# mahfuzalhasan/WaveFormer

Measured on AMD Instinct MI355X. Metric: 128³×4 volumes/sec fwd (1/2/4/8 MI355X) + Dice Δ vs reference, higher is better.
Workload: dtype bf16x3; 1 GPU; MultiscaleTransformer (WaveFormer encoder) forward, 128^3x4 crops; global_batch=8, per_gpu_batch=8, precision=bf16x3, parallelism=replicas x1 (no data-path collective), hip_graph=True

## Files before the change

waveformer_amd/csrc/pw2.hip:

```cpp
#include <algorithm>

#include "gemm_common.hpp"

namespace wf {

namespace pw2 {
constexpr int K = 96, N = 384, KS = K / 32, NT = N / 16;
constexpr int RB = K * 2;
constexpr int PLANE = N * RB;
}

__device__ __forceinline__ int pw2_chunk(int n, int o) {
  const int f = (0x1E >> (2 * ((n >> 2) & 3))) & 3;
  return (o & ~3) | ((o & 3) ^ f);
}

template <int P, int NW>
__global__ __launch_bounds__(64 * NW, 1) void pw2_res_kernel(GemmArgs g) {
  using namespace pw2;
  constexpr bool SPLIT = P == PREC_SPLIT;
  constexpr int NPL = SPLIT ? 2 : 1;
  extern __shared__ __attribute__((aligned(16))) unsigned char smem[];
  float* ew = reinterpret_cast<float*>(smem + NPL * PLANE);
  float* eb = ew + N;
  float* bs = eb + N;
  float* aw = bs + N;
  float* ab = aw + K;
  const int tid = threadIdx.x, lane = tid & 63, wid = tid >> 6;
  const int l15 = lane & 15, g4 = lane >> 4;

  for (int it = tid; it < NPL * N * (K / 8); it += 64 * NW) {
    const int pr = it / (K / 8), o = it - pr * (K / 8);
    const int n = pr % N;
    *reinterpret_cast<bf16x8*>(smem + pr * RB + 16 * pw2_chunk(n, o)) =
        *reinterpret_cast<const bf16x8*>(g.w + (int64_t)pr * K + 8 * o);
  }
  for (int i = tid; i < N; i += 64 * NW) {
    ew[i] = 0.5f * g.e_ln_w[i];
    eb[i] = 0.5f * g.e_ln_b[i];
    bs[i] = g.bias ? g.bias[i] : 0.f;
  }
  const bool aln = g.a_ln == LN_GIVEN;
  for (int i = tid; i < K; i += 64 * NW) {
    aw[i] = aln ? g.a_ln_w[i] : 1.f;
    ab[i] = aln ? g.a_ln_b[i] : 0.f;
  }
  __syncthreads();

  const int M = (int)g.M;
  const int ntiles = (M + 15) >> 4;
  const float* xa = reinterpret_cast<const float*>(g.a_src);
  f32x4 an[KS][2];
  float mn = 0.f, rn = 1.f;
  auto aload = [&](int tile) {
    const int row = min(tile * 16 + l15, M - 1);
    const float* p = xa + (int64_t)row * K + 8 * g4;
#pragma unroll
    for (int ks = 0; ks < KS; ++ks) {
      an[ks][0] = *reinterpret_cast<const f32x4*>(p + 32 * ks);
      an[ks][1] = *reinterpret_cast<const f32x4*>(p + 32 * ks + 4);
    }
    if (aln) {
      mn = g.a_stats[2 * row];
      rn = g.a_stats[2 * row + 1];
    }
  };
  int tile = blockIdx.x * NW + wid;
  const int stride = gridDim.x * NW;
  if (tile < ntiles) aload(tile);
  const int wlane = l15 * RB + 16 * ((g4 ^ ((0x1E >> (2 * ((l15 >> 2) & 3))) & 3)));
  for (; tile < ntiles; tile += stride) {
    bf16x8 ah[KS], al[KS];
    const float mu = mn, rs = rn;
#pragma unroll
    for (int ks = 0; ks < KS; ++ks) {
      const int k = 32 * ks + 8 * g4;
#pragma unroll
      for (int hq = 0; hq < 2; ++hq) {
        f32x4 v = an[ks][hq];
        if (aln) {
          const f32x4 lw = *reinterpret_cast<const f32x4*>(aw + k + 4 * hq);
          const f32x4 lb = *reinterpret_cast<const f32x4*>(ab + k + 4 * hq);
          v = (v - mu) * rs * lw + lb;
        }
        uint32_t h0, h1, l0, l1;
        split_pair<P>(v[0], v[1], h0, l0);
        split_pair<P>(v[2], v[3], h1, l1);
        ah[ks][4 * hq] = (short)(h0 & 0xFFFF);
        ah[ks][4 * hq + 1] = (short)(h0 >> 16);
        ah[ks][4 * hq + 2] = (short)(h1 & 0xFFFF);
        ah[ks][4 * hq + 3] = (short)(h1 >> 16);
        al[ks][4 * hq] = (short)(l0 & 0xFFFF);
        al[ks][4 * hq + 1] = (short)(l0 >> 16);
        al[ks][4 * hq + 2] = (short)(l1 & 0xFFFF);
        al[ks][4 * hq + 3] = (short)(l1 >> 16);
      }
    }
    if (tile + stride < ntiles) aload(tile + stride);

    int wb = wlane;
    asm volatile("" : "+v"(wb));
    const unsigned char* Wb = smem + wb;
    f32x4 acc[NT];
#pragma unroll
    for (int t = 0; t < NT; ++t) acc[t] = f32x4{0.f, 0.f, 0.f, 0.f};
#pragma unroll
    for (int ks = 0; ks < KS; ++ks) {
#pragma unroll
      for (int t = 0; t < NT; ++t) {
        const int wo = t * 16 * RB + 64 * ks;
        const bf16x8 bh = *reinterpret_cast<const bf16x8*>(Wb + wo);
        const bf16x8 bl = SPLIT ? *reinterpret_cast<const bf16x8*>(Wb + PLANE + wo) : bh;
        acc[t] = mma3<P>(acc[t], bh, bl, ah[ks], al[ks]);
        if (t % 4 == 3) __builtin_amdgcn_sched_barrier(0);
      }
    }

#pragma unroll
    for (int t = 0; t < NT; ++t) acc[t] += *reinterpret_cast<const f32x4*>(bs + 16 * t + 4 * g4);
    float part[8];
#pragma unroll
    for (int w = 0; w < 8; ++w) part[w] = tile_sum<3>(acc + 3 * w);
    const float mean =
        (((part[0] + part[1]) + (part[2] + part[3])) + ((part[4] + part[5]) + (part[6] + part[7]))) *
        (1.f / N);
#pragma unroll
    for (int w = 0; w < 8; ++w) part[w] = tile_sqdev<3>(acc + 3 * w, mean);
    const float rstd = rsqrtf(
        (((part[0] + part[1]) + (part[2] + part[3])) + ((part[4] + part[5]) + (part[6] + part[7]))) *
            (1.f / N) + g.e_eps);
    const int row = tile * 16 + l15;
    float* o = reinterpret_cast<float*>(g.out) + (int64_t)min(row, M - 1) * g.ldo + 4 * g4;
#pragma unroll
    for (int t = 0; t < NT; ++t) {
      const f32x4 lw = *reinterpret_cast<const f32x4*>(ew + 16 * t + 4 * g4);
      const f32x4 lb = *reinterpret_cast<const f32x4*>(eb + 16 * t + 4 * g4);
      const f32x4 v = gelu_half4((acc[t] - mean) * rstd * lw + lb);
      if (row < M) *reinterpret_cast<f32x4*>(o + 16 * t) = v;
      if (t % 4 == 3) __builtin_amdgcn_sched_barrier(0);
    }
  }
}

int try_launch_pw2_resident(const GemmArgs& g, hipStream_t s) {
  using namespace pw2;
  static const bool off = getenv("WF_PW2_RES") != nullptr && getenv("WF_PW2_RES")[0] == '0';
  if (off || g.epi != EPI_LN_GELU || g.a_map != MAP_IDENTITY || g.a_bf16 || g.a_gelu ||
      !(g.a_ln == LN_NONE || g.a_ln == LN_GIVEN) || g.K != K || g.N != N || g.a_C != K ||
      g.out_bf16 || g.ldo < N || g.ldo % 4 != 0 || (g.prec != PREC_SPLIT && g.prec != PREC_FP16) ||
      g.M < 1 || g.M >= ((int64_t)1 << 31) - 16)
    return 0;
  constexpr int NW = 8;
  const bool split = g.prec == PREC_SPLIT;
  const size_t lds = (size_t)(split ? 2 : 1) * PLANE + (size_t)(3 * N + 2 * K) * 4;
  void (*kern)(GemmArgs) = split ? pw2_res_kernel<PREC_SPLIT, NW> : pw2_res_kernel<PREC_FP16, NW>;
  set_max_lds(reinterpret_cast<const void*>(kern), (int)lds);
  const int64_t ntiles = (g.M + 15) / 16;
  const unsigned gx = (unsigned)std::min<int64_t>(cdiv(ntiles, NW), 256);
  hipLaunchKernelGGL(kern, dim3(gx), dim3(64 * NW), lds, s, g);
  return 1;
}

}
```

waveformer_amd/csrc/gemm.hip:

```cpp
#include "gemm_common.hpp"

namespace wf {

__device__ __forceinline__ void load8(const void* src, int is_bf16, int64_t off, float (&v)[8]) {
  if (is_bf16) load8f<true>(src, off, v);
  else load8f<false>(src, off, v);
}

struct RowSource {
  const GemmArgs& g;
  int64_t pos;
  __device__ RowSource(const GemmArgs& g_, int64_t m) : g(g_), pos(0) {
    if (g.a_map == MAP_WINDOW) {
      const int ws = g.mws;
      const int N = ws * ws * ws;
      const int nWd = g.mD / ws, nWh = g.mH / ws, nWw = g.mW / ws;
      const int64_t bw = m / N;
      const int t = (int)(m - bw * N);
      const int nW = nWd * nWh * nWw;
      const int b = (int)(bw / nW);
      int wi = (int)(bw - (int64_t)b * nW);
      const int wx = wi % nWw;
      wi /= nWw;
      const int wy = wi % nWh;
      const int wz = wi / nWh;
      const int tx = t % ws, ty = (t / ws) % ws, tz = t / (ws * ws);
      pos = (((int64_t)b * g.mD + wz * ws + tz) * g.mH + wy * ws + ty) * g.mW + wx * ws + tx;
    } else if (g.a_map == MAP_MERGE) {
      const int d = g.mD >> 1, h = g.mH >> 1, w = g.mW >> 1;
      int64_t r = m;
      const int x = (int)(r % w);
      r /= w;
      const int y = (int)(r % h);
      r /= h;
      const int z = (int)(r % d);
      const int b = (int)(r / d);
      pos = (((int64_t)b * g.mD + 2 * z) * g.mH + 2 * y) * g.mW + 2 * x;
    } else {
      pos = m;
    }
  }
  __device__ int64_t offset(int k) const {
    if (g.a_map == MAP_MERGE) {
      const int seg = k / g.a_C;
      const int c = k - seg * g.a_C;
      const int o = (g.merge_code >> (4 * seg)) & 0xF;
      const int64_t p = pos + (((int64_t)((o >> 2) & 1) * g.mH + ((o >> 1) & 1)) * g.mW) +
                        (o & 1);
      return p * g.a_C + c;
    }
    return pos * (int64_t)(g.a_C * g.a_nseg) + k;
  }
};

template <int TPR>
__device__ __forceinline__ float tpr_sum(float v) {
#pragma unroll
  for (int o = TPR / 2; o > 0; o >>= 1) v += __shfl_xor(v, o, 64);
  return v;
}

template <int BM, int P>
__global__ __launch_bounds__(256) void gemm_ares_kernel(GemmArgs g) {
  constexpr bool SPLIT = P == PREC_SPLIT;
  extern __shared__ __attribute__((aligned(16))) char smem[];
  constexpr int TPR = 256 / BM;
  constexpr int MT = BM / 16;
  const int K = g.K, N = g.N;
  const int K32 = (K + 31) & ~31;
  const int KP = K32 + 8;
  const int NP = N + 4;
  const size_t abytes = ((size_t)BM * KP * 2 + 15) & ~(size_t)15;
  uint16_t* A = reinterpret_cast<uint16_t*>(smem);
  uint16_t* Alo = reinterpret_cast<uint16_t*>(smem + abytes);
  float* R = reinterpret_cast<float*>(smem + (SPLIT ? 2 : 1) * abytes);
  float* st = R + (size_t)BM * NP;

  const int tid = threadIdx.x, lane = tid & 63, wid = tid >> 6;
  const int64_t m0 = (int64_t)blockIdx.x * BM;

  {
    const int r = tid / TPR, q = tid % TPR;
    const int64_t m = m0 + r;
    const bool mv = m < g.M;
    float mean = 0.f, rstd = 1.f;
    if (g.a_ln == LN_GIVEN) {
      if (mv) {
        mean = g.a_stats[2 * m];
        rstd = g.a_stats[2 * m + 1];
      }
    } else if (g.a_ln == LN_COMPUTE) {
      RowSource rs(g, mv ? m : 0);
      float s = 0.f;
      for (int ch = q; ch < K / 8; ch += TPR) {
        float v[8];
        load8(g.a_src, g.a_bf16, rs.offset(ch * 8), v);
#pragma unroll
        for (int j = 0; j < 8; ++j) s += v[j];
      }
      mean = tpr_sum<TPR>(s) / (float)K;
      float sq = 0.f;
      for (int ch = q; ch < K / 8; ch += TPR) {
        float v[8];
        load8(g.a_src, g.a_bf16, rs.offset(ch * 8), v);
#pragma unroll
        for (int j = 0; j < 8; ++j) {
          const float dlt = v[j] - mean;
          sq += dlt * dlt;
        }
      }
      rstd = rsqrtf(tpr_sum<TPR>(sq) / (float)K + g.a_eps);
    } else if (g.a_ln == LN_PARTIAL) {
      const int np = g.a_np;
      const float* ps = g.a_stats + (mv ? m : 0) * np * 2;
      float s = 0.f;
      for (int c = q; c < np; c += TPR) s += ps[2 * c];
      mean = tpr_sum<TPR>(s) / (float)np;
      const float ng = (float)(K / np);
      float sq = 0.f;
      for (int c = q; c < np; c += TPR) {
        const float d = ps[2 * c] - mean;
        sq += ps[2 * c + 1] + ng * d * d;
      }
      rstd = rsqrtf(tpr_sum<TPR>(sq) / (float)K + g.a_eps);
    }
    if (q == 0) {
      st[2 * r] = mean;
      st[2 * r + 1] = rstd;
    }
  }
  __syncthreads();
  {
    const int KC = K32 / 8;
    for (int item = tid; item < BM * KC; item += 256) {
      const int r = item / KC, ch = item - r * KC;
      const int64_t m = m0 + r;
      bf16x8 o = {0, 0, 0, 0, 0, 0, 0, 0}, olo = {0, 0, 0, 0, 0, 0, 0, 0};
      if (m < g.M && ch * 8 < K) {
        RowSource rs(g, m);
        float v[8];
        load8(g.a_src, g.a_bf16, rs.offset(ch * 8), v);
        if (g.a_ln != LN_NONE) {
          const float mean = st[2 * r], rstd = st[2 * r + 1];
          const f32x4* gw = reinterpret_cast<const f32x4*>(g.a_ln_w + ch * 8);
          const f32x4* gb = reinterpret_cast<const f32x4*>(g.a_ln_b + ch * 8);
          const f32x4 w0 = gw[0], w1 = gw[1], b0 = gb[0], b1 = gb[1];
          const float wv[8] = {w0.x, w0.y, w0.z, w0.w, w1.x, w1.y, w1.z, w1.w};
          const float bv[8] = {b0.x, b0.y, b0.z, b0.w, b1.x, b1.y, b1.z, b1.w};
#pragma unroll
          for (int j = 0; j < 8; ++j) v[j] = (v[j] - mean) * rstd * wv[j] + bv[j];
        }
        if (g.a_gelu) {
          gelu_erf8(v);
        }
#pragma unroll
        for (int j = 0; j < 8; ++j) {
          const uint16_t hi = op_cvt<P>(v[j]);
          o[j] = (short)hi;
          if (SPLIT) olo[j] = op_lo<P>(v[j], hi);
        }
      }
      *reinterpret_cast<bf16x8*>(A + (size_t)r * KP + ch * 8) = o;
      if (SPLIT) *reinterpret_cast<bf16x8*>(Alo + (size_t)r * KP + ch * 8) = olo;
    }
  }
  __syncthreads();

  const int kq = 8 * (lane >> 4);
  for (int n0 = 0; n0 < N; n0 += 64) {
    const int n = n0 + wid * 16 + (lane & 15);
    const bool nv = n < N;
    const uint16_t* wrow = g.w + (int64_t)(nv ? n : 0) * K;
    const uint16_t* wlo = wrow + (int64_t)N * K;
    f32x4 acc[MT];
#pragma unroll
    for (int mt = 0; mt < MT; ++mt) acc[mt] = f32x4{0, 0, 0, 0};
    const bf16x8 z8 = {0, 0, 0, 0, 0, 0, 0, 0};
    bf16x8 bnext = z8, blnext = z8;
    if (nv && kq < K) {
      bnext = *reinterpret_cast<const bf16x8*>(wrow + kq);
      if (SPLIT) blnext = *reinterpret_cast<const bf16x8*>(wlo + kq);
    }
    for (int k0 = 0; k0 < K32; k0 += 32) {
      const bf16x8 b = bnext, bl = blnext;
      bnext = z8;
      blnext = z8;
      if (nv && k0 + 32 + kq < K) {
        bnext = *reinterpret_cast<const bf16x8*>(wrow + k0 + 32 + kq);
        if (SPLIT) blnext = *reinterpret_cast<const bf16x8*>(wlo + k0 + 32 + kq);
      }
#pragma unroll
      for (int mt = 0; mt < MT; ++mt) {
        const size_t aoff = (size_t)(mt * 16 + (lane & 15)) * KP + k0 + kq;
        const bf16x8 a = *reinterpret_cast<const bf16x8*>(A + aoff);
        if (SPLIT) {
          const bf16x8 al = *reinterpret_cast<const bf16x8*>(Alo + aoff);
          acc[mt] = mma32<P>(al, b, acc[mt]);
          acc[mt] = mma32<P>(a, bl, acc[mt]);
        }
        acc[mt] = mma32<P>(a, b, acc[mt]);
      }
    }
    if (nv) {
#pragma unroll
      for (int mt = 0; mt < MT; ++mt)
#pragma unroll
        for (int i = 0; i < 4; ++i) R[(size_t)(mt * 16 + 4 * (lane >> 4) + i) * NP + n] = acc[mt][i];
    }
  }
  __syncthreads();

  const int N4 = N >> 2;
  if (g.epi == EPI_LN_GELU) {
    const int r = tid / TPR, q = tid % TPR;
    float s = 0.f;
    for (int c4 = q; c4 < N4; c4 += TPR) {
      f32x4 v = *reinterpret_cast<const f32x4*>(R + (size_t)r * NP + 4 * c4);
      if (g.bias) v += reinterpret_cast<const f32x4*>(g.bias)[c4];
      s += (v.x + v.y) + (v.z + v.w);
    }
    const float mean = tpr_sum<TPR>(s) / (float)N;
    float sq = 0.f;
    for (int c4 = q; c4 < N4; c4 += TPR) {
      f32x4 v = *reinterpret_cast<const f32x4*>(R + (size_t)r * NP + 4 * c4);
      if (g.bias) v += reinterpret_cast<const f32x4*>(g.bias)[c4];
      v -= mean;
      sq += (v.x * v.x + v.y * v.y) + (v.z * v.z + v.w * v.w);
    }
    const float rstd = rsqrtf(tpr_sum<TPR>(sq) / (float)N + g.e_eps);
    __syncthreads();
    if (q == 0) {
      st[2 * r] = mean;
      st[2 * r + 1] = rstd;
    }
    __syncthreads();
  }
  for (int item = tid; item < BM * N4; item += 256) {
    const int r = item / N4, c4 = item - r * N4;
    const int64_t m = m0 + r;
    if (m >= g.M) continue;
    f32x4 v = *reinterpret_cast<const f32x4*>(R + (size_t)r * NP + 4 * c4);
    if (g.bias) v += reinterpret_cast<const f32x4*>(g.bias)[c4];
    if (g.epi == EPI_LN_GELU) {
      const f32x4 lw = reinterpret_cast<const f32x4*>(g.e_ln_w)[c4];
      const f32x4 lb = reinterpret_cast<const f32x4*>(g.e_ln_b)[c4];
      v = (v - st[2 * r]) * st[2 * r + 1] * lw + lb;
      v = gelu_erf4(v);
    } else if (g.epi == EPI_RESID) {
      const f32x4 xr = reinterpret_cast<const f32x4*>(g.r_x + m * (int64_t)N)[c4];
      const float bs = g.r_scale ? g.r_scale[m / g.rows_per_sample] : 1.f;
      float mean = 0.f, rstd = 1.f;
      if (g.r_stats) {
        mean = g.r_stats[2 * m];
        rstd = g.r_stats[2 * m + 1];
      }
      v = resid_epilogue(v, xr, mean, rstd, g.r_ln_w + 4 * c4, g.r_ln_b + 4 * c4, bs,
                         g.r_stats != nullptr);
    }
    store4(g.out, g.out_bf16 != 0, m * g.ldo, 4 * c4, v);
  }
}

static size_t gemm_lds_bytes(int BM, int K, int N, bool split) {
  const size_t K32 = (size_t)((K + 31) & ~31);
  const size_t a = ((size_t)BM * (K32 + 8) * 2 + 15) & ~(size_t)15;
  return (split ? 2 : 1) * a + (size_t)BM * (N + 4) * 4 + (size_t)BM * 2 * 4;
}

int launch_gemm(const GemmArgs& g, hipStream_t s, const char* who) {
  if (g.K <= 0 || g.K % 8 != 0) return fail(WF_E_SHAPE, std::string(who) + ": K must be a positive multiple of 8");
  if (g.N <= 0 || g.N % 4 != 0) return fail(WF_E_SHAPE, std::string(who) + ": N must be a positive multiple of 4");
  if (g.a_C % 8 != 0) return fail(WF_E_SHAPE, std::string(who) + ": channels must be a multiple of 8");
  if (g.M <= 0) return WF_OK;
  if (g.o_pstats) {
    if (g.epi == EPI_STORE && !g.out_bf16 && !g.a_bf16 && try_launch_gemm_kc(g, s))
      return check_launch(who);
    return fail(WF_E_SHAPE, std::string(who) + ": LN-partial epilogue needs the gemm_kc shape");
  }
  if (try_launch_gemm_lnw(g, s)) return check_launch(who);
  if (try_launch_gemm_rows(g, s, true)) return check_launch(who);
  if (try_launch_gemm_kc(g, s)) return check_launch(who);
  const bool split = g.prec == PREC_SPLIT;
  int BM = 64;
  while (BM > 16 && gemm_lds_bytes(BM, g.K, g.N, split) > 80 * 1024) BM >>= 1;
  const size_t lds = gemm_lds_bytes(BM, g.K, g.N, split);
  if (lds > 160 * 1024) return fail(WF_E_SHAPE, std::string(who) + ": K/N too large for the LDS tile");
  const unsigned blocks = (unsigned)cdiv(g.M, BM);
  auto go = [&](auto kern) {
    if (lds > 64 * 1024)
      set_max_lds(reinterpret_cast<const void*>(kern), (int)lds);
    hipLaunchKernelGGL(kern, dim3(blocks), dim3(256), lds, s, g);
  };
  gemm_with_prec(g.prec, false, [&](auto P, auto) {
    switch (BM) {
      case 64: go(gemm_ares_kernel<64, P()>); break;
      case 32: go(gemm_ares_kernel<32, P()>); break;
      default: go(gemm_ares_kernel<16, P()>); break;
    }
  });
  return check_launch(who);
}

}
```

waveformer_amd/csrc/kernels.hpp:

```cpp
#pragma once
#include "wf_common.hpp"

namespace wf {

enum Prec { PREC_BF16 = 0, PREC_SPLIT = 1, PREC_FP16 = 2 };

typedef _Float16 f16x4 __attribute__((ext_vector_type(4)));
typedef _Float16 f16x8 __attribute__((ext_vector_type(8)));
__device__ __forceinline__ uint16_t f2h(float f) { return __builtin_bit_cast(uint16_t, (_Float16)f); }

template <int P>
__device__ __forceinline__ uint16_t op_cvt(float x) {
  if constexpr (P == PREC_FP16) return f2h(x);
  else return f2bf(x);
}
template <int P>
__device__ __forceinline__ short op_lo(float x, uint16_t hi) {
  if constexpr (P == PREC_SPLIT) return (short)f2bf(x - bf2f(hi));
  else return (short)0;
}
template <int P>
__device__ __forceinline__ f32x4 mma32(bf16x8 a, bf16x8 b, f32x4 c) {
  if constexpr (P == PREC_FP16)
    return __builtin_amdgcn_mfma_f32_16x16x32_f16(__builtin_bit_cast(f16x8, a),
                                                  __builtin_bit_cast(f16x8, b), c, 0, 0, 0);
  else return __builtin_amdgcn_mfma_f32_16x16x32_bf16(a, b, c, 0, 0, 0);
}
template <int P>
__device__ __forceinline__ f32x4 mma16(bf16x4 a, bf16x4 b, f32x4 c) {
  if constexpr (P == PREC_FP16)
    return __builtin_amdgcn_mfma_f32_16x16x16f16(__builtin_bit_cast(f16x4, a),
                                                 __builtin_bit_cast(f16x4, b), c, 0, 0, 0);
  else return __builtin_amdgcn_mfma_f32_16x16x16bf16_1k(a, b, c, 0, 0, 0);
}
template <int P>
__device__ __forceinline__ f32x4 mma3(f32x4 acc, const bf16x8& w_hi, const bf16x8& w_lo,
                                      const bf16x8& a_hi, const bf16x8& a_lo) {
  if constexpr (P == PREC_SPLIT) {
    acc = mma32<P>(w_hi, a_lo, acc);
    acc = mma32<P>(w_lo, a_hi, acc);
  }
  return mma32<P>(w_hi, a_hi, acc);
}
typedef __bf16 bf16v2 __attribute__((ext_vector_type(2)));
template <int P>
__device__ __forceinline__ void split_pair(float y0, float y1, uint32_t& hi, uint32_t& lo) {
  if constexpr (P == PREC_SPLIT) {
    uint32_t m0, m1;
    asm("s_mov_b32 %0, 0xbf80" : "=s"(m0));
    asm("s_mov_b32 %0, 0xbf800000" : "=s"(m1));
    const bf16v2 h = bf16v2{(__bf16)y0, (__bf16)y1};
    const float r0 = __builtin_amdgcn_fdot2_f32_bf16(h, __builtin_bit_cast(bf16v2, m0), y0, false);
    const float r1 = __builtin_amdgcn_fdot2_f32_bf16(h, __builtin_bit_cast(bf16v2, m1), y1, false);
    hi = __builtin_bit_cast(uint32_t, h);
    lo = __builtin_bit_cast(uint32_t, bf16v2{(__bf16)r0, (__bf16)r1});
  } else {
    hi = (uint32_t)op_cvt<P>(y0) | ((uint32_t)op_cvt<P>(y1) << 16);
    lo = 0;
  }
}
template <int P>
__device__ __forceinline__ void split4(f32x4 v, bf16x4& h, bf16x4& l) {
  uint32_t h0, h1, l0, l1;
  split_pair<P>(v[0], v[1], h0, l0);
  split_pair<P>(v[2], v[3], h1, l1);
  h = __builtin_bit_cast(bf16x4, u32x2{h0, h1});
  l = __builtin_bit_cast(bf16x4, u32x2{l0, l1});
}
template <int P>
__device__ __forceinline__ void split8(const float (&x)[8], bf16x8& h, bf16x8& l) {
  uint32_t hw[4], lw[4];
#pragma unroll
  for (int j = 0; j < 4; ++j) split_pair<P>(x[2 * j], x[2 * j + 1], hw[j], lw[j]);
  h = __builtin_bit_cast(bf16x8, u32x4{hw[0], hw[1], hw[2], hw[3]});
  l = __builtin_bit_cast(bf16x8, u32x4{lw[0], lw[1], lw[2], lw[3]});
}
__host__ __device__ constexpr bool store32(int p) { return p != PREC_BF16; }
inline bool valid_prec(int p) { return p == PREC_BF16 || p == PREC_SPLIT || p == PREC_FP16; }

enum RowMap { MAP_IDENTITY = 0, MAP_WINDOW = 1, MAP_MERGE = 2, MAP_LEVELS = 3 };
constexpr int WF_MAX_LEVELS = 4;
enum LnMode { LN_NONE = 0, LN_GIVEN = 1, LN_COMPUTE = 2, LN_PARTIAL = 3 };
enum EpiMode { EPI_STORE = 0, EPI_LN_GELU = 1, EPI_RESID = 2, EPI_SUBVOXEL = 3 };

struct GemmArgs {
  int prec;
  const void* a_src;
  int a_bf16;
  int a_C;
  int a_nseg;
  int a_map;
  int mB, mD, mH, mW, mws;
  int merge_code;
  int a_ln;
  const float* a_stats;
  int a_np;
  const float* a_ln_w;
  const float* a_ln_b;
  float a_eps;
  int a_gelu;
  const uint16_t* w;
  int64_t M;
  int N, K;
  int epi;
  const float* bias;
  void* out;
  int out_bf16;
  int64_t ldo;
  const float* e_ln_w;
  const float* e_ln_b;
  float e_eps;
  const float* r_x;
  const float* r_stats;
  const float* r_ln_w;
  const float* r_ln_b;
  const float* r_scale;
  int64_t rows_per_sample;
  float* o_pstats;
  float* kpart;
  int64_t kpart_bytes;
  int ksplit;
  const float* lv_src[WF_MAX_LEVELS];
  int lv_row0[WF_MAX_LEVELS];
  int lv_D[WF_MAX_LEVELS], lv_H[WF_MAX_LEVELS], lv_W[WF_MAX_LEVELS];
};

int launch_gemm(const GemmArgs& g, hipStream_t s, const char* who);
int gemm_kc_pick_nt(const GemmArgs& g);
int launch_instnorm_partial(const float* x, int64_t ldx, int64_t B, int64_t C, int64_t P,
                            double* acc, hipStream_t s);
int try_launch_gemm_rows(const GemmArgs& g, hipStream_t s, bool single_chunk_only);

int launch_attn_core(const void* qkv, const float* bias, void* out, float* lse, int64_t Bw,
                     int N, int heads, int hd, float scale, int prec, hipStream_t s,
                     int table_ws = 0, int64_t pair_windows = -1, const GemmArgs* fused = nullptr);
bool attn_tbl_pair_loop(int64_t wh);

int launch_dwconv_ln_gelu(const void* in, const float* w, const float* b, const float* ln_w,
                          const float* ln_b, float eps, void* out, int B, int Hd, int D, int H,
                          int W, int prec, hipStream_t s);
int launch_dwconv3d(const void* in, const float* w, const float* b, void* out, float* pstats,
                    int B, int Hd, int D, int H, int W, int prec, hipStream_t s,
                    double* cstats = nullptr, const float* ln1_stats = nullptr,
                    const float* ln1_w = nullptr, const float* ln1_b = nullptr, int flip = 0);
int launch_ln_stats_finalize(const float* pstats, int np, int group, float eps, float* out,
                             int64_t M, hipStream_t s);
constexpr int DW_STAT_GROUP = 32;
int try_launch_gemm_kc(const GemmArgs& g, hipStream_t s);
int try_launch_merge_resident(const GemmArgs& g, hipStream_t s);
int try_launch_pw2_resident(const GemmArgs& g, hipStream_t s);
int try_launch_gemm_lnw(const GemmArgs& g, hipStream_t s);
bool gemm_lnw_wide_shape(const GemmArgs& g);

}

#include "ffn_dwfc_common.hpp"
```

Baseline: 1268 volumes/s.

## Split pw2 row tile's N columns across wave pairs with LDS LayerNorm reduction

After: 1271 volumes/s, median of 5. No clear change (+0.2%).

```diff
diff --git a/waveformer_amd/csrc/pw2.hip b/waveformer_amd/csrc/pw2.hip
--- a/waveformer_amd/csrc/pw2.hip
+++ b/waveformer_amd/csrc/pw2.hip
@@ -15,19 +15,32 @@
   return (o & ~3) | ((o & 3) ^ f);
 }
 
+constexpr int pw2_lds_bytes(int npl, int nw) {
+  return npl * pw2::PLANE + (3 * pw2::N + 2 * pw2::K) * 4 + 2 * nw * 16 * 4;
+}
+
 template <int P, int NW>
 __global__ __launch_bounds__(64 * NW, 1) void pw2_res_kernel(GemmArgs g) {
   using namespace pw2;
   constexpr bool SPLIT = P == PREC_SPLIT;
   constexpr int NPL = SPLIT ? 2 : 1;
+  constexpr int NP = NW / 2;
+  constexpr int HT = NT / 2;
+  static_assert(NW % 2 == 0 && HT % 3 == 0, "a wave holds whole 3-tile moment partials");
+  static_assert(pw2_lds_bytes(NPL, NW) <= 160 * 1024, "LDS of one CU");
   extern __shared__ __attribute__((aligned(16))) unsigned char smem[];
   float* ew = reinterpret_cast<float*>(smem + NPL * PLANE);
   float* eb = ew + N;
   float* bs = eb + N;
   float* aw = bs + N;
   float* ab = aw + K;
-  const int tid = threadIdx.x, lane = tid & 63, wid = tid >> 6;
+  float* xs = ab + K;
+  float* xq = xs + NW * 16;
+  const int tid = threadIdx.x, lane = tid & 63;
+  const int wid = __builtin_amdgcn_readfirstlane(tid >> 6);
   const int l15 = lane & 15, g4 = lane >> 4;
+  const int pair = wid >> 1, half = wid & 1;
+  const int cb = half * (HT * 16);
 
   for (int it = tid; it < NPL * N * (K / 8); it += 64 * NW) {
     const int pr = it / (K / 8), o = it - pr * (K / 8);
@@ -65,16 +78,22 @@
       rn = g.a_stats[2 * row + 1];
     }
   };
-  int tile = blockIdx.x * NW + wid;
-  const int stride = gridDim.x * NW;
-  if (tile < ntiles) aload(tile);
-  const int wlane = l15 * RB + 16 * ((g4 ^ ((0x1E >> (2 * ((l15 >> 2) & 3))) & 3)));
-  for (; tile < ntiles; tile += stride) {
+  const int stride = gridDim.x * NP;
+  const int niter = (ntiles + stride - 1) / stride;
+  int tile = blockIdx.x * NP + pair;
+  aload(min(tile, ntiles - 1));
+#pragma unroll
+  for (int ks = 0; ks < KS; ++ks) asm volatile("" : "+v"(an[ks][0]), "+v"(an[ks][1]));
+  asm volatile("" : "+v"(mn), "+v"(rn));
+  const int wlane = (cb + l15) * RB + 16 * ((g4 ^ ((0x1E >> (2 * ((l15 >> 2) & 3))) & 3)));
+  for (int it = 0; it < niter; ++it, tile += stride) {
     bf16x8 ah[KS], al[KS];
     const float mu = mn, rs = rn;
+    int kq = 8 * g4, cq = cb + 4 * g4;
+    asm volatile("" : "+v"(kq), "+v"(cq));
 #pragma unroll
     for (int ks = 0; ks < KS; ++ks) {
-      const int k = 32 * ks + 8 * g4;
+      const int k = 32 * ks + kq;
 #pragma unroll
       for (int hq = 0; hq < 2; ++hq) {
         f32x4 v = an[ks][hq];
@@ -96,18 +115,18 @@
         al[ks][4 * hq + 3] = (short)(l1 >> 16);
       }
     }
-    if (tile + stride < ntiles) aload(tile + stride);
+    if (it + 1 < niter) aload(min(tile + stride, ntiles - 1));
 
     int wb = wlane;
     asm volatile("" : "+v"(wb));
     const unsigned char* Wb = smem + wb;
-    f32x4 acc[NT];
+    f32x4 acc[HT];
 #pragma unroll
-    for (int t = 0; t < NT; ++t) acc[t] = f32x4{0.f, 0.f, 0.f, 0.f};
+    for (int t = 0; t < HT; ++t) acc[t] = f32x4{0.f, 0.f, 0.f, 0.f};
 #pragma unroll
     for (int ks = 0; ks < KS; ++ks) {
 #pragma unroll
-      for (int t = 0; t < NT; ++t) {
+      for (int t = 0; t < HT; ++t) {
         const int wo = t * 16 * RB + 64 * ks;
         const bf16x8 bh = *reinterpret_cast<const bf16x8*>(Wb + wo);
         const bf16x8 bl = SPLIT ? *reinterpret_cast<const bf16x8*>(Wb + PLANE + wo) : bh;
@@ -117,26 +136,32 @@
     }
 
 #pragma unroll
-    for (int t = 0; t < NT; ++t) acc[t] += *reinterpret_cast<const f32x4*>(bs + 16 * t + 4 * g4);
-    float part[8];
+    for (int t = 0; t < HT; ++t) acc[t] += *reinterpret_cast<const f32x4*>(bs + cq + 16 * t);
+    float part[4];
 #pragma unroll
-    for (int w = 0; w < 8; ++w) part[w] = tile_sum<3>(acc + 3 * w);
-    const float mean =
-        (((part[0] + part[1]) + (part[2] + part[3])) + ((part[4] + part[5]) + (part[6] + part[7]))) *
-        (1.f / N);
+    for (int w = 0; w < 4; ++w) part[w] = tile_sum<3>(acc + 3 * w);
+    if (g4 == 0) xs[wid * 16 + l15] = (part[0] + part[1]) + (part[2] + part[3]);
+    __syncthreads();
+    const float mean = (xs[(2 * pair) * 16 + l15] + xs[(2 * pair + 1) * 16 + l15]) * (1.f / N);
 #pragma unroll
-    for (int w = 0; w < 8; ++w) part[w] = tile_sqdev<3>(acc + 3 * w, mean);
+    for (int w = 0; w < 4; ++w) part[w] = tile_sqdev<3>(acc + 3 * w, mean);
+    if (g4 == 0) xq[wid * 16 + l15] = (part[0] + part[1]) + (part[2] + part[3]);
+    __syncthreads();
     const float rstd = rsqrtf(
-        (((part[0] + part[1]) + (part[2] + part[3])) + ((part[4] + part[5]) + (part[6] + part[7]))) *
-            (1.f / N) + g.e_eps);
-    const int row = tile * 16 + l15;
-    float* o = reinterpret_cast<float*>(g.out) + (int64_t)min(row, M - 1) * g.ldo + 4 * g4;
+        (xq[(2 * pair) * 16 + l15] + xq[(2 * pair + 1) * 16 + l15]) * (1.f / N) + g.e_eps);
+    const int tl = min(tile, ntiles - 1);
+    const int vrows = tile < ntiles ? min(16, M - tl * 16) : 0;
+    const __amdgpu_buffer_rsrc_t orsrc = __builtin_amdgcn_make_buffer_rsrc(
+        reinterpret_cast<float*>(g.out) + (int64_t)tl * 16 * g.ldo, 0, vrows * g.ldo * 4,
+        0x00020000);
+    const int oo = (l15 * g.ldo + cb + 4 * g4) * 4;
 #pragma unroll
-    for (int t = 0; t < NT; ++t) {
-      const f32x4 lw = *reinterpret_cast<const f32x4*>(ew + 16 * t + 4 * g4);
-      const f32x4 lb = *reinterpret_cast<const f32x4*>(eb + 16 * t + 4 * g4);
+    for (int t = 0; t < HT; ++t) {
+      const f32x4 lw = *reinterpret_cast<const f32x4*>(ew + cq + 16 * t);
+      const f32x4 lb = *reinterpret_cast<const f32x4*>(eb + cq + 16 * t);
       const f32x4 v = gelu_half4((acc[t] - mean) * rstd * lw + lb);
-      if (row < M) *reinterpret_cast<f32x4*>(o + 16 * t) = v;
+      __builtin_amdgcn_raw_buffer_store_b128(__builtin_bit_cast(u32x4, v), orsrc, oo + 64 * t, 0,
+                                             0);
       if (t % 4 == 3) __builtin_amdgcn_sched_barrier(0);
     }
   }
@@ -148,15 +173,16 @@
   if (off || g.epi != EPI_LN_GELU || g.a_map != MAP_IDENTITY || g.a_bf16 || g.a_gelu ||
       !(g.a_ln == LN_NONE || g.a_ln == LN_GIVEN) || g.K != K || g.N != N || g.a_C != K ||
       g.out_bf16 || g.ldo < N || g.ldo % 4 != 0 || (g.prec != PREC_SPLIT && g.prec != PREC_FP16) ||
-      g.M < 1 || g.M >= ((int64_t)1 << 31) - 16)
+      g.M < 1 || g.M >= ((int64_t)1 << 31) - 16 ||
+      g.ldo > (1 << 20))
     return 0;
-  constexpr int NW = 8;
+  constexpr int NW = 16;
   const bool split = g.prec == PREC_SPLIT;
-  const size_t lds = (size_t)(split ? 2 : 1) * PLANE + (size_t)(3 * N + 2 * K) * 4;
+  const size_t lds = (size_t)pw2_lds_bytes(split ? 2 : 1, NW);
   void (*kern)(GemmArgs) = split ? pw2_res_kernel<PREC_SPLIT, NW> : pw2_res_kernel<PREC_FP16, NW>;
   set_max_lds(reinterpret_cast<const void*>(kern), (int)lds);
   const int64_t ntiles = (g.M + 15) / 16;
-  const unsigned gx = (unsigned)std::min<int64_t>(cdiv(ntiles, NW), 256);
+  const unsigned gx = (unsigned)std::min<int64_t>(cdiv(ntiles, NW / 2), 256);
   hipLaunchKernelGGL(kern, dim3(gx), dim3(64 * NW), lds, s, g);
   return 1;
 }
```

## Add alternating-column GEMM kernel that overlaps A-transform with MFMA work

Applied to the files above, without the earlier changes.

New measurement: 1269 volumes/s before, 1278 volumes/s after, median of 6. Within noise of the previous version (+0.7%).

```diff
diff --git a/waveformer_amd/csrc/gemm.hip b/waveformer_amd/csrc/gemm.hip
--- a/waveformer_amd/csrc/gemm.hip
+++ b/waveformer_amd/csrc/gemm.hip
@@ -279,6 +279,7 @@
   }
   if (try_launch_gemm_lnw(g, s)) return check_launch(who);
   if (try_launch_gemm_rows(g, s, true)) return check_launch(who);
+  if (try_launch_gemm_ac(g, s)) return check_launch(who);
   if (try_launch_gemm_kc(g, s)) return check_launch(who);
   const bool split = g.prec == PREC_SPLIT;
   int BM = 64;
diff --git a/waveformer_amd/csrc/gemm_ac.hip b/waveformer_amd/csrc/gemm_ac.hip
--- /dev/null
+++ b/waveformer_amd/csrc/gemm_ac.hip
@@ -0,0 +1,251 @@
+#include <algorithm>
+#include <cstdlib>
+
+#include "gemm_common.hpp"
+
+namespace wf {
+
+constexpr int AC_BK = 32;
+constexpr int AC_KP = AC_BK + WF_LDS_KPAD;
+
+template <int RW, int CW, int NT>
+struct AcCfg {
+  static constexpr int WAVES = RW * CW, NTHR = 64 * WAVES, ROWS = 16 * RW;
+  static constexpr int SPAN = CW * NT * 16;
+  static constexpr int WITEMS = SPAN * (AC_BK / 8);
+  static constexpr int WPT = (WITEMS + NTHR - 1) / NTHR;
+  static_assert(CW == 2, "the k loop alternates two column groups");
+};
+
+template <int RW, int CW, int NT, int P, int MAP, int EPI>
+__global__ __launch_bounds__(64 * RW * CW) void gemm_ac_kernel(GemmArgs g) {
+  typedef AcCfg<RW, CW, NT> C;
+  constexpr bool SPLIT = P == PREC_SPLIT;
+  constexpr int SPAN = C::SPAN, ROWS = C::ROWS, NPL = SPLIT ? 2 : 1;
+  extern __shared__ __attribute__((aligned(16))) uint16_t Wl[];
+  const int K = g.K, N = g.N;
+  const int M = (int)g.M;
+  const int nks = (K + AC_BK - 1) / AC_BK;
+  const int nks2 = (nks + 1) & ~1;
+  const int c0 = blockIdx.y * SPAN;
+  const int tid = threadIdx.x, lane = tid & 63;
+  const int wid = __builtin_amdgcn_readfirstlane(tid >> 6);
+  const int l15 = lane & 15, g4 = lane >> 4;
+  const int wr = wid % RW, wc = wid / RW;
+  const int rbase = blockIdx.x * ROWS + wr * 16;
+  uint16_t* Al = Wl + (size_t)2 * NPL * SPAN * AC_KP;
+  float* lnw = reinterpret_cast<float*>(Al + (size_t)2 * NPL * ROWS * AC_KP);
+  const int nln = (nks2 + 1) * AC_BK;
+  float* lnb = lnw + nln;
+  float* st = lnb + nln;
+
+  typedef bf16x8 WRegs[NPL][C::WPT];
+  WRegs wst[2];
+  auto wfetch = [&](int ks, WRegs& dst) {
+#pragma unroll
+    for (int j = 0; j < C::WPT; ++j) {
+      const int i = min(j * C::NTHR + tid, C::WITEMS - 1);
+      const int n = c0 + (i >> 2), k = ks * AC_BK + 8 * (i & 3);
+      const int64_t off = (int64_t)min(n, N - 1) * K + min(k, K - 8);
+      dst[0][j] = *reinterpret_cast<const bf16x8*>(g.w + off);
+      if (SPLIT) dst[NPL - 1][j] = *reinterpret_cast<const bf16x8*>(g.w + (int64_t)N * K + off);
+    }
+  };
+  auto wcommit = [&](int buf, const WRegs& src) {
+#pragma unroll
+    for (int j = 0; j < C::WPT; ++j) {
+      const int i = j * C::NTHR + tid;
+      if (i < C::WITEMS) {
+#pragma unroll
+        for (int pl = 0; pl < NPL; ++pl)
+          *reinterpret_cast<bf16x8*>(Wl + ((size_t)(buf * NPL + pl) * SPAN + (i >> 2)) * AC_KP +
+                                     8 * (i & 3)) = src[pl][j];
+      }
+    }
+  };
+
+  const int arow = min(rbase + l15, M - 1);
+  const RowMapper<MAP> rm(g, arow);
+  float mean = 0.f, rstd = 1.f;
+  if (g.a_ln != LN_NONE) {
+    if (wc == 0) {
+      if (g.a_ln == LN_GIVEN) {
+        mean = g.a_stats[2 * arow];
+        rstd = g.a_stats[2 * arow + 1];
+      }
+      if (g.a_ln == LN_COMPUTE) {
+        float v0[8];
+        load8f<false>(g.a_src, rm.offset(g, 0), v0);
+        const float sh = v0[0];
+        float s = 0.f, q = 0.f;
+        ln_row_batches<false>(g.a_src, K / 8, g4, [&](int k) { return rm.offset(g, k); },
+                              [&](float x, float mk) {
+                                const float d = (x - sh) * mk;
+                                s += d;
+                                q += d * d;
+                              });
+        s = xsum16(s);
+        s = xsum32(s);
+        q = xsum16(q);
+        q = xsum32(q);
+        const float ms = s / (float)K;
+        mean = sh + ms;
+        rstd = rsqrtf(fmaxf(q / (float)K - ms * ms, 0.f) + g.a_eps);
+      } else if (g.a_ln == LN_PARTIAL) {
+        ln_partial_combine(g.a_stats + (int64_t)arow * g.a_np * 2, g.a_np, K, g.a_eps, g4, mean, rstd);
+      }
+      if (g4 == 0) {
+        st[2 * (wr * 16 + l15)] = mean;
+        st[2 * (wr * 16 + l15) + 1] = rstd;
+      }
+    }
+    for (int i = tid; i < nln; i += C::NTHR) {
+      lnw[i] = i < K ? g.a_ln_w[i] : 0.f;
+      lnb[i] = i < K ? g.a_ln_b[i] : 0.f;
+    }
+    __syncthreads();
+    mean = st[2 * (wr * 16 + l15)];
+    rstd = st[2 * (wr * 16 + l15) + 1];
+  }
+
+  f32x4 acc[NT];
+#pragma unroll
+  for (int t = 0; t < NT; ++t) acc[t] = f32x4{0, 0, 0, 0};
+
+  float an[8];
+  auto afetch = [&](int ks) {
+    const int k = min(min(ks, nks - 1) * AC_BK + 8 * g4, K - 8);
+    load8f<false>(g.a_src, rm.offset(g, k), an);
+  };
+  auto xform = [&](int ks) {
+    const int k = ks * AC_BK + 8 * g4;
+    const bool kv = k < K;
+    float v[8];
+#pragma unroll
+    for (int j = 0; j < 8; ++j) v[j] = an[j];
+    bf16x8 ah, al;
+    a_fragment<P>(v, mean, rstd, lnw, lnb, k, kv, g.a_ln != LN_NONE, g.a_gelu != 0, ah, al);
+    uint16_t* dst = Al + ((size_t)(ks & 1) * NPL * ROWS + wr * 16 + l15) * AC_KP + 8 * g4;
+    *reinterpret_cast<bf16x8*>(dst) = ah;
+    if (SPLIT) *reinterpret_cast<bf16x8*>(dst + (size_t)ROWS * AC_KP) = al;
+  };
+
+  typedef std::integral_constant<int, 0> Slot0;
+  typedef std::integral_constant<int, 1> Slot1;
+  auto run = [&](auto role) {
+    constexpr int R = decltype(role)::value;
+    wfetch(0, wst[0]);
+    afetch(R);
+    wfetch(min(1, nks - 1), wst[1]);
+    wcommit(0, wst[0]);
+    if constexpr (R == 0) {
+      xform(0);
+      afetch(2);
+    }
+    __syncthreads();
+    auto kbody = [&](int ks, auto slot) {
+      constexpr int S = decltype(slot)::value;
+      wfetch(min(ks + 2, nks - 1), wst[S]);
+      if constexpr (R == (S ^ 1)) {
+        xform(ks + 1);
+        afetch(ks + 3);
+      }
+      const uint16_t* Ab = Al + ((size_t)S * NPL * ROWS + wr * 16 + l15) * AC_KP + 8 * g4;
+      const bf16x8 ah = *reinterpret_cast<const bf16x8*>(Ab);
+      const bf16x8 al = SPLIT ? *reinterpret_cast<const bf16x8*>(Ab + (size_t)ROWS * AC_KP) : ah;
+      const uint16_t* Wb = Wl + (size_t)S * NPL * SPAN * AC_KP;
+#pragma unroll
+      for (int t = 0; t < NT; ++t) {
+        const int wo = ((R * NT + t) * 16 + l15) * AC_KP + 8 * g4;
+        const bf16x8 bh = *reinterpret_cast<const bf16x8*>(Wb + wo);
+        const bf16x8 bl = SPLIT ? *reinterpret_cast<const bf16x8*>(Wb + SPAN * AC_KP + wo) : bh;
+        acc[t] = mma3<P>(acc[t], bh, bl, ah, al);
+        if (t % 4 == 3) __builtin_amdgcn_sched_barrier(0);
+      }
+      wcommit(S ^ 1, wst[S ^ 1]);
+      __syncthreads();
+    };
+#pragma unroll 1
+    for (int ks = 0; ks < nks; ks += 2) {
+      kbody(ks, Slot0{});
+      kbody(ks + 1, Slot1{});
+    }
+  };
+  if (wc == 0) run(Slot0{});
+  else run(Slot1{});
+
+  const int cw0 = c0 + wc * NT * 16;
+  const int row = rbase + l15;
+  const bool rv = row < M;
+  const int rowc = min(row, M - 1);
+  if (g.bias) {
+#pragma unroll
+    for (int t = 0; t < NT; ++t)
+      acc[t] += *reinterpret_cast<const f32x4*>(g.bias + min(cw0 + t * 16 + 4 * g4, N - 4));
+  }
+  float rm_ = 0.f, rs_ = 1.f, bs = 1.f;
+  if (EPI == EPI_RESID) {
+    if (g.r_stats) {
+      rm_ = g.r_stats[2 * rowc];
+      rs_ = g.r_stats[2 * rowc + 1];
+    }
+    if (g.r_scale) bs = g.r_scale[rowc / (int)g.rows_per_sample];
+  }
+#pragma unroll
+  for (int t = 0; t < NT; ++t) {
+    const int col = cw0 + t * 16 + 4 * g4;
+    const int colc = min(col, N - 4);
+    f32x4 v = acc[t];
+    if (EPI == EPI_RESID) {
+      const f32x4 xr = *reinterpret_cast<const f32x4*>(g.r_x + (int64_t)rowc * N + colc);
+      v = resid_epilogue(v, xr, rm_, rs_, g.r_ln_w + colc, g.r_ln_b + colc, bs, g.r_stats != nullptr);
+    }
+    if (rv && col < N) store4(g.out, false, (int64_t)row * g.ldo, col, v);
+    if (t % 2 == 1) __builtin_amdgcn_sched_barrier(0);
+  }
+}
+
+typedef AcCfg<8, 2, 6> AcTile;
+
+static size_t ac_lds_bytes(const GemmArgs& g) {
+  const int nks2 = ((int)cdiv(g.K, AC_BK) + 1) & ~1;
+  const size_t npl = g.prec == PREC_SPLIT ? 2 : 1;
+  return 2 * npl * (AcTile::SPAN + AcTile::ROWS) * AC_KP * 2 + (size_t)2 * (nks2 + 1) * AC_BK * 4 +
+         (size_t)AcTile::ROWS * 2 * 4;
+}
+
+static bool gemm_ac_takes(const GemmArgs& g) {
+  if (!store32(g.prec) || g.a_bf16 || g.out_bf16 || g.o_pstats) return false;
+  if (g.a_map == MAP_LEVELS || !gemm_known_callsite(g)) return false;
+  if (g.epi != EPI_STORE && g.epi != EPI_RESID) return false;
+  if (g.N % AcTile::SPAN != 0 || g.K % AC_BK != 0) return false;
+  if (!((g.N == AcTile::SPAN && g.K >= 768) || (g.N >= 6 * AcTile::SPAN && g.K >= 384))) return false;
+  if (g.M < 1 || g.M >= ((int64_t)1 << 31) - AcTile::ROWS) return false;
+  if (g.kpart && g.a_gelu && g.K >= 1536) return false;
+  return ac_lds_bytes(g) <= 160 * 1024;
+}
+
+template <int MAP, int EPI>
+static void go_ac(const GemmArgs& g, hipStream_t s) {
+  typedef AcTile C;
+  void (*kern)(GemmArgs) = g.prec == PREC_SPLIT ? gemm_ac_kernel<8, 2, 6, PREC_SPLIT, MAP, EPI>
+                                                : gemm_ac_kernel<8, 2, 6, PREC_FP16, MAP, EPI>;
+  const size_t lds = ac_lds_bytes(g);
+  if (lds > 64 * 1024) set_max_lds(reinterpret_cast<const void*>(kern), (int)lds);
+  GemmArgs ga = g;
+  ga.ksplit = 1;
+  const dim3 grid((unsigned)cdiv(g.M, C::ROWS), (unsigned)(g.N / C::SPAN));
+  hipLaunchKernelGGL(kern, grid, dim3(C::NTHR), lds, s, ga);
+}
+
+int try_launch_gemm_ac(const GemmArgs& g, hipStream_t s) {
+  static const bool off = getenv("WF_GEMM_AC") != nullptr && getenv("WF_GEMM_AC")[0] == '0';
+  if (off || !gemm_ac_takes(g)) return 0;
+  if (g.a_map == MAP_WINDOW) go_ac<MAP_WINDOW, EPI_STORE>(g, s);
+  else if (g.a_map == MAP_MERGE) go_ac<MAP_MERGE, EPI_STORE>(g, s);
+  else if (g.epi == EPI_RESID) go_ac<MAP_IDENTITY, EPI_RESID>(g, s);
+  else go_ac<MAP_IDENTITY, EPI_STORE>(g, s);
+  return 1;
+}
+
+}
diff --git a/waveformer_amd/csrc/kernels.hpp b/waveformer_amd/csrc/kernels.hpp
--- a/waveformer_amd/csrc/kernels.hpp
+++ b/waveformer_amd/csrc/kernels.hpp
@@ -147,6 +147,7 @@
                              int64_t M, hipStream_t s);
 constexpr int DW_STAT_GROUP = 32;
 int try_launch_gemm_kc(const GemmArgs& g, hipStream_t s);
+int try_launch_gemm_ac(const GemmArgs& g, hipStream_t s);
 int try_launch_merge_resident(const GemmArgs& g, hipStream_t s);
 int try_launch_pw2_resident(const GemmArgs& g, hipStream_t s);
 int try_launch_gemm_lnw(const GemmArgs& g, hipStream_t s);
```
